# facebookresearch/jepa

Measured on NVIDIA H100. Metric: clips/sec ViT-L/16 16x224^2 synthetic V-JEPA pre-training step, higher is better.
Workload: dtype bf16

## Files before the change

### __graft_entry__.py

```python
import os
import sys

ROOT = os.path.dirname(os.path.abspath(__file__))
if ROOT not in sys.path:
    sys.path.insert(0, ROOT)


def build():
    from jepa_b200 import build as b
    b.build()
    import subprocess
    subprocess.check_call(["make", "-s", "-C", os.path.join(ROOT, "tests", "native"), "all", "test_xattn",
                           "test_gemm_sched"])
    import jepa_b200
    from jepa_b200 import _lib
    _lib.load()
    import oracle.vjepa_oracle


def smoke():
    import torch
    sys.path.insert(0, os.path.join(ROOT, "tests"))
    sys.path.insert(0, os.path.join(ROOT, "tests", "golden"))
    from parity_util import run_c1_step_cuda, run_c1_step_oracle, compare_step
    assert torch.cuda.is_available(), "smoke() needs cuda:0"
    dev = torch.device("cuda:0")
    got = run_c1_step_cuda(dev, batch=1, depth_limit=2)
    ref = run_c1_step_oracle(batch=1, depth_limit=2)
    compare_step(got, ref, verbose=True)
    print("smoke OK: loss", got["loss_jepa"], "oracle", ref["loss_jepa"])


if __name__ == "__main__":
    build()
    if len(sys.argv) > 1 and sys.argv[1] == "smoke":
        smoke()
```

### jepa_b200/csrc/attn_bwd.cu

```cuda
#include <stdlib.h>

#include "attn_common.cuh"
#include "vjepa_b200.h"

namespace vj {

constexpr int kBwdThreads = 384;
constexpr int kBwdStream = 64;
constexpr int kBwdStages = 3;

struct AttnBwdParams {
  const int* cu_seqlens;
  const float* lse2;
  const float* delta;
  __nv_bfloat16* dqkv;
  int H, T;
  float scale, scale_log2;
};

template <int HD>
struct BwdCfg {
  using A = AttnCfg<HD>;
  static constexpr int RES = A::template tile_bytes<128>();
  static constexpr int STR = A::template tile_bytes<kBwdStream>();
  static constexpr int T0 = 0, T1 = RES;
  static constexpr int S_OFF = 2 * RES;
  static constexpr int STAT_OFF = S_OFF + kBwdStages * 2 * STR;
  static constexpr int STAT = 2 * kBwdStream * 4;
  static constexpr int BAR_OFF = STAT_OFF + kBwdStages * STAT;
  static constexpr int SMEM_BYTES = BAR_OFF + 8 * (1 + 2 * kBwdStages) + 1024;
  static_assert(SMEM_BYTES <= 232448, "attention backward shared memory budget exceeded");
};

__global__ void __launch_bounds__(256) attn_delta_kernel(const __nv_bfloat16* __restrict__ o,
                                                         const __nv_bfloat16* __restrict__ dout,
                                                         float* __restrict__ delta, int T, int H, int HD) {
  const int lane = threadIdx.x & 31;
  const int wpb = blockDim.x >> 5;
  const int D = H * HD;
  const int nvec = D >> 3;
  const int lanes_per_head = HD >> 3;
  for (long long t = (long long)blockIdx.x * wpb + (threadIdx.x >> 5); t < T; t += (long long)gridDim.x * wpb) {
    for (int c = lane; c < ((nvec + 31) / 32) * 32; c += 32) {
      float s = 0.f;
      if (c < nvec) {
        const uint4 a = *reinterpret_cast<const uint4*>(o + t * D + c * 8);
        const uint4 b = *reinterpret_cast<const uint4*>(dout + t * D + c * 8);
        s = bf16_lo(a.x) * bf16_lo(b.x) + bf16_hi(a.x) * bf16_hi(b.x) + bf16_lo(a.y) * bf16_lo(b.y) +
            bf16_hi(a.y) * bf16_hi(b.y) + bf16_lo(a.z) * bf16_lo(b.z) + bf16_hi(a.z) * bf16_hi(b.z) +
            bf16_lo(a.w) * bf16_lo(b.w) + bf16_hi(a.w) * bf16_hi(b.w);
      }
      for (int o2 = lanes_per_head >> 1; o2 > 0; o2 >>= 1) s += __shfl_xor_sync(0xffffffffu, s, o2);
      if (c < nvec && (lane % lanes_per_head) == 0) delta[(long long)((c * 8) / HD) * T + t] = s;
    }
  }
}

template <int HD, bool DKV>
__global__ void __launch_bounds__(kBwdThreads, 1)
attn_bwd_kernel(const __grid_constant__ CUtensorMap tmRes, const __grid_constant__ CUtensorMap tmStr,
                const __grid_constant__ CUtensorMap tmDO, const AttnBwdParams p) {
  using B = BwdCfg<HD>;
  extern __shared__ uint8_t smem_raw[];
  uint8_t* smem = reinterpret_cast<uint8_t*>((reinterpret_cast<uintptr_t>(smem_raw) + 1023) & ~uintptr_t(1023));

  const int seq = blockIdx.y, head = blockIdx.z;
  const int row_begin = p.cu_seqlens[seq];
  const int len = p.cu_seqlens[seq + 1] - row_begin;
  const int t0 = blockIdx.x * 128;
  if (t0 >= len) return;
  const int n_it = (len + kBwdStream - 1) / kBwdStream;
  const int HHD = p.H * HD;

  uint64_t* bars = reinterpret_cast<uint64_t*>(smem + B::BAR_OFF);
  const uint32_t bar_res = smem_u32(bars + 0);
  const uint32_t full0 = smem_u32(bars + 1);
  const uint32_t empty0 = smem_u32(bars + 1 + kBwdStages);
  const uint32_t sT0 = smem_u32(smem + B::T0), sT1 = smem_u32(smem + B::T1), sS = smem_u32(smem + B::S_OFF);
  const uint32_t sStat = smem_u32(smem + B::STAT_OFF);
  const float* lse_h = p.lse2 + (long long)head * p.T + row_begin;
  const float* del_h = p.delta + (long long)head * p.T + row_begin;
  const int wg = threadIdx.x >> 7;
  const int lane = threadIdx.x & 31;

  if (threadIdx.x == 0) {
    mbar_init(bar_res, 1);
    for (int st = 0; st < kBwdStages; ++st) {
      mbar_init(full0 + 8 * st, DKV ? 32 : 1);
      mbar_init(empty0 + 8 * st, 8);
    }
    fence_mbar_init();
  }
  __syncthreads();

  if (wg == 0) {
    setmaxnreg_dec<40>();
    if (threadIdx.x < 32) {
      if (lane == 0) {
        mbar_expect_tx(bar_res, 2 * B::RES);
        if (DKV) {
          attn_load_tile<HD, 128>(sT0, &tmRes, bar_res, HHD + head * HD, row_begin + t0);
          attn_load_tile<HD, 128>(sT1, &tmRes, bar_res, 2 * HHD + head * HD, row_begin + t0);
        } else {
          attn_load_tile<HD, 128>(sT0, &tmRes, bar_res, head * HD, row_begin + t0);
          attn_load_tile<HD, 128>(sT1, &tmDO, bar_res, head * HD, row_begin + t0);
        }
      }
      for (int i = 0; i < n_it; ++i) {
        const int st = i % kBwdStages;
        const uint32_t a = sS + st * 2 * B::STR, b = a + B::STR, bar = full0 + 8 * st;
        const int c0 = i * kBwdStream;
        mbar_wait(empty0 + 8 * st, ((i / kBwdStages) & 1) ^ 1);
        if (DKV) {
#pragma unroll
          for (int k = 0; k < kBwdStream / 32; ++k) {
            const int col = c0 + 32 * k + lane;
            const uint32_t dst = sStat + st * B::STAT + (32 * k + lane) * 4;
            sts32f(dst, col < len ? lse_h[col] : 0.f);
            sts32f(dst + B::STAT / 2, col < len ? del_h[col] : 0.f);
          }
        }
        if (lane == 0) {
          mbar_expect_tx(bar, 2 * B::STR);
          if (DKV) {
            attn_load_tile<HD, kBwdStream>(a, &tmStr, bar, head * HD, row_begin + c0);
            attn_load_tile<HD, kBwdStream>(b, &tmDO, bar, head * HD, row_begin + c0);
          } else {
            attn_load_tile<HD, kBwdStream>(a, &tmStr, bar, HHD + head * HD, row_begin + c0);
            attn_load_tile<HD, kBwdStream>(b, &tmStr, bar, 2 * HHD + head * HD, row_begin + c0);
          }
        } else if (DKV) {
          mbar_arrive(bar);
        }
      }
    }
    return;
  }

  setmaxnreg_inc<232>();
  const int cw = wg - 1;
  const int r = cw * 64 + ((threadIdx.x >> 5) & 3) * 16 + (lane >> 2);
  float acc0[HD / 2], acc1[HD / 2];
#pragma unroll
  for (int i = 0; i < HD / 2; ++i) { acc0[i] = 0.f; acc1[i] = 0.f; }
  float row_lse[2], row_del[2];
  if (!DKV) {
#pragma unroll
    for (int h = 0; h < 2; ++h) {
      const int q = t0 + r + 8 * h;
      row_lse[h] = q < len ? lse_h[q] : 0.f;
      row_del[h] = q < len ? del_h[q] : 0.f;
    }
  }
  mbar_wait(bar_res, 0);
  for (int i = 0; i < n_it; ++i) {
    const int st = i % kBwdStages;
    const uint32_t sa = sS + st * 2 * B::STR, sb = sa + B::STR;
    const int c0 = i * kBwdStream;
    mbar_wait(full0 + 8 * st, (i / kBwdStages) & 1);
    float x[kBwdStream / 2], y[kBwdStream / 2];
    wgmma_fence();
#pragma unroll
    for (int kk = 0; kk < HD / 16; ++kk)
      wgmma_ss<kBwdStream, 0, 0>(x, attn_kmajor_desc<HD, 128>(sT0, cw * 64, kk), attn_kmajor_desc<HD, kBwdStream>(sa, 0, kk),
                                 kk > 0);
#pragma unroll
    for (int kk = 0; kk < HD / 16; ++kk)
      wgmma_ss<kBwdStream, 0, 0>(y, attn_kmajor_desc<HD, 128>(sT1, cw * 64, kk), attn_kmajor_desc<HD, kBwdStream>(sb, 0, kk),
                                 kk > 0);
    wgmma_commit();
    wgmma_wait<0>();
    wgmma_fence_regs(x);
    wgmma_fence_regs(y);

#pragma unroll
    for (int c = 0; c < kBwdStream / 8; ++c)
#pragma unroll
      for (int e = 0; e < 2; ++e) {
        const int col = 8 * c + 2 * (lane & 3) + e;
        const bool col_ok = c0 + col < len;
        float cl = 0.f, cd = 0.f;
        if (DKV) {
          cl = lds32f(sStat + st * B::STAT + col * 4);
          cd = lds32f(sStat + st * B::STAT + B::STAT / 2 + col * 4);
        }
#pragma unroll
        for (int h = 0; h < 2; ++h) {
          const float l2 = DKV ? cl : row_lse[h], dl = DKV ? cd : row_del[h];
          float& pv = x[4 * c + 2 * h + e];
          float& dv = y[4 * c + 2 * h + e];
          pv = col_ok ? ex2_approx(fmaf(pv, p.scale_log2, -l2)) : 0.f;
          dv = pv * (dv - dl);
        }
      }

    wgmma_fence_regs(acc0);
    wgmma_fence_regs(acc1);
    wgmma_fence();
#pragma unroll
    for (int kk = 0; kk < kBwdStream / 16; ++kk) {
      uint32_t a[4];
      if (DKV) {
        acc_to_afrag(x, kk, a);
        wgmma_rs<HD, 1>(acc0, a, attn_mnmajor_desc<HD, kBwdStream>(sb, kk), 1);
        acc_to_afrag(y, kk, a);
        wgmma_rs<HD, 1>(acc1, a, attn_mnmajor_desc<HD, kBwdStream>(sa, kk), 1);
      } else {
        acc_to_afrag(y, kk, a);
        wgmma_rs<HD, 1>(acc0, a, attn_mnmajor_desc<HD, kBwdStream>(sa, kk), 1);
      }
    }
    wgmma_commit();
    wgmma_wait<0>();
    wgmma_fence_regs(acc0);
    wgmma_fence_regs(acc1);
    __syncwarp();
    if (lane == 0) mbar_arrive(empty0 + 8 * st);
  }

  __nv_bfloat16* rows = p.dqkv + (long long)(row_begin + t0) * 3 * HHD + head * HD;
  if (DKV) {
    store_frag_bf16<HD>(acc1, p.scale, rows + HHD, 3LL * HHD, r, len - t0);
    store_frag_bf16<HD>(acc0, 1.0f, rows + 2 * HHD, 3LL * HHD, r, len - t0);
  } else {
    store_frag_bf16<HD>(acc0, p.scale, rows, 3LL * HHD, r, len - t0);
  }
}

template <int HD>
static int launch_attn_bwd(const void* qkv, const void* out, const void* dout, const float* lse2, float* delta,
                           void* dqkv, const int* cu, int nseq, int max_len, int H, int T, float scale, cudaStream_t s) {
  using C = AttnCfg<HD>;
  using B = BwdCfg<HD>;
  CUtensorMap tq128, tq64, tdo128, tdo64;
  const uint64_t W = (uint64_t)3 * H * HD;
  int rc = make_tmap_2d(&tq128, qkv, 0, W, T, W * 2, C::BOX_INNER, 128, C::TMAP_SWIZZLE);
  if (!rc) rc = make_tmap_2d(&tq64, qkv, 0, W, T, W * 2, C::BOX_INNER, kBwdStream, C::TMAP_SWIZZLE);
  if (!rc) rc = make_tmap_2d(&tdo128, dout, 0, (uint64_t)H * HD, T, (uint64_t)H * HD * 2, C::BOX_INNER, 128, C::TMAP_SWIZZLE);
  if (!rc) rc = make_tmap_2d(&tdo64, dout, 0, (uint64_t)H * HD, T, (uint64_t)H * HD * 2, C::BOX_INNER, kBwdStream,
                             C::TMAP_SWIZZLE);
  if (rc) return rc;
  auto kdkv = attn_bwd_kernel<HD, true>;
  auto kdq = attn_bwd_kernel<HD, false>;
  static bool configured = false;
  if (!configured) {
    VJ_CUDA(cudaFuncSetAttribute(kdkv, cudaFuncAttributeMaxDynamicSharedMemorySize, B::SMEM_BYTES));
    VJ_CUDA(cudaFuncSetAttribute(kdq, cudaFuncAttributeMaxDynamicSharedMemorySize, B::SMEM_BYTES));
    configured = true;
  }
  {
    int g = (T + 7) / 8;
    const int cap = num_sms() * 8;
    if (g > cap) g = cap;
    attn_delta_kernel<<<g, 256, 0, s>>>(reinterpret_cast<const __nv_bfloat16*>(out),
                                        reinterpret_cast<const __nv_bfloat16*>(dout), delta, T, H, HD);
    VJ_CUDA(cudaGetLastError());
    vj::count_launch(1);
  }
  AttnBwdParams p;
  p.cu_seqlens = cu; p.lse2 = lse2; p.delta = delta; p.dqkv = reinterpret_cast<__nv_bfloat16*>(dqkv);
  p.H = H; p.T = T; p.scale = scale; p.scale_log2 = scale * 1.4426950408889634f;
  dim3 grid((max_len + 127) / 128, nseq, H);
  kdkv<<<grid, kBwdThreads, B::SMEM_BYTES, s>>>(tq128, tq64, tdo64, p);
  VJ_CUDA(cudaGetLastError());
  kdq<<<grid, kBwdThreads, B::SMEM_BYTES, s>>>(tq128, tq64, tdo128, p);
  VJ_CUDA(cudaGetLastError());
  vj::count_launch(2);
  return 0;
}

}

extern "C" int vj_attn_bwd(const void* qkv, const void* out, const void* dout, const float* lse2, float* delta_ws,
                           void* dqkv, float* dq_acc_ws, const int* cu_seqlens, int nseq, int max_len, int H, int HD,
                           int T, float scale, void* stream_) {
  using namespace vj;
  (void)dq_acc_ws;
  cudaStream_t s = reinterpret_cast<cudaStream_t>(stream_);
  VJ_CHECK_ARG(qkv && out && dout && lse2 && delta_ws && dqkv && cu_seqlens, "vj_attn_bwd: null pointer");
  VJ_CHECK_ARG(nseq > 0 && max_len > 0 && H > 0 && T > 0, "vj_attn_bwd: empty problem");
  switch (HD) {
    case 32: return launch_attn_bwd<32>(qkv, out, dout, lse2, delta_ws, dqkv, cu_seqlens, nseq, max_len, H, T, scale, s);
    case 64: return launch_attn_bwd<64>(qkv, out, dout, lse2, delta_ws, dqkv, cu_seqlens, nseq, max_len, H, T, scale, s);
    case 128: return launch_attn_bwd<128>(qkv, out, dout, lse2, delta_ws, dqkv, cu_seqlens, nseq, max_len, H, T, scale, s);
    default: set_error("vj_attn_bwd: head dim %d unsupported (32/64/128)", HD); return -1;
  }
}
```

### jepa_b200/csrc/attn_fwd.cu

```cuda
#include <stdlib.h>

#include "attn_common.cuh"
#include "vjepa_b200.h"

namespace vj {

constexpr int kFwdThreads = 384;
constexpr int kFwdKV = 128;
constexpr int kFwdStages = 3;

struct AttnFwdParams {
  const int* cu_seqlens;
  __nv_bfloat16* out;
  float* lse2;
  int H, T;
  long long ld_out;
  float scale_log2;
};

template <int HD>
struct FwdCfg {
  using A = AttnCfg<HD>;
  static constexpr int TILE = A::template tile_bytes<128>();
  static constexpr int Q_OFF = 0;
  static constexpr int K_OFF = TILE;
  static constexpr int V_OFF = K_OFF + kFwdStages * TILE;
  static constexpr int BAR_OFF = V_OFF + kFwdStages * TILE;
  static constexpr int SMEM_BYTES = BAR_OFF + 8 * (1 + 2 * kFwdStages) + 1024;
  static_assert(SMEM_BYTES <= 232448, "attention forward shared memory budget exceeded");
};

VJ_DEVINL void pingpong_wait_turn(int cw) { named_bar_sync(1 + cw, 256); }
VJ_DEVINL void pingpong_pass_turn(int cw) { named_bar_arrive(2 - cw, 256); }

template <int HD>
__global__ void __launch_bounds__(kFwdThreads, 1)
attn_fwd_kernel(const __grid_constant__ CUtensorMap tmQKV, const AttnFwdParams p) {
  using F = FwdCfg<HD>;
  extern __shared__ uint8_t smem_raw[];
  uint8_t* smem = reinterpret_cast<uint8_t*>((reinterpret_cast<uintptr_t>(smem_raw) + 1023) & ~uintptr_t(1023));

  const int seq = blockIdx.y, head = blockIdx.z;
  const int row_begin = p.cu_seqlens[seq];
  const int len = p.cu_seqlens[seq + 1] - row_begin;
  const int q0 = blockIdx.x * 128;
  if (q0 >= len) return;
  const int n_kv = (len + kFwdKV - 1) / kFwdKV;

  uint64_t* bars = reinterpret_cast<uint64_t*>(smem + F::BAR_OFF);
  const uint32_t bar_q = smem_u32(bars + 0);
  const uint32_t full0 = smem_u32(bars + 1);
  const uint32_t empty0 = smem_u32(bars + 1 + kFwdStages);
  const uint32_t sQ = smem_u32(smem + F::Q_OFF), sK = smem_u32(smem + F::K_OFF), sV = smem_u32(smem + F::V_OFF);
  const int HHD = p.H * HD;
  const int wg = threadIdx.x >> 7;

  if (threadIdx.x == 0) {
    mbar_init(bar_q, 1);
    for (int st = 0; st < kFwdStages; ++st) {
      mbar_init(full0 + 8 * st, 1);
      mbar_init(empty0 + 8 * st, 8);
    }
    fence_mbar_init();
    tma_prefetch_desc(&tmQKV);
  }
  __syncthreads();

  if (wg == 0) {
    setmaxnreg_dec<40>();
    if (threadIdx.x == 0) {
      mbar_expect_tx(bar_q, F::TILE);
      attn_load_tile<HD, 128>(sQ, &tmQKV, bar_q, head * HD, row_begin + q0);
      for (int j = 0; j < n_kv; ++j) {
        const int st = j % kFwdStages;
        mbar_wait(empty0 + 8 * st, ((j / kFwdStages) & 1) ^ 1);
        const uint32_t fb = full0 + 8 * st;
        mbar_expect_tx(fb, 2 * F::TILE);
        attn_load_tile<HD, 128>(sK + st * F::TILE, &tmQKV, fb, HHD + head * HD, row_begin + j * kFwdKV);
        attn_load_tile<HD, 128>(sV + st * F::TILE, &tmQKV, fb, 2 * HHD + head * HD, row_begin + j * kFwdKV);
      }
    }
    return;
  }

  setmaxnreg_inc<232>();
  const int cw = wg - 1;
  const int lane = threadIdx.x & 31;
  const int r = cw * 64 + ((threadIdx.x >> 5) & 3) * 16 + (lane >> 2);
  float o[HD / 2];
#pragma unroll
  for (int i = 0; i < HD / 2; ++i) o[i] = 0.f;
  float m_run[2] = {-INFINITY, -INFINITY}, l_run[2] = {0.f, 0.f};
  float s[kFwdKV / 2];
  uint32_t pf[kFwdKV / 16][4];
  if (cw == 1) pingpong_pass_turn(cw);

  auto issue_s = [&](int st) {
#pragma unroll
    for (int kk = 0; kk < HD / 16; ++kk)
      wgmma_ss<kFwdKV, 0, 0>(s, attn_kmajor_desc<HD, 128>(sQ, cw * 64, kk),
                             attn_kmajor_desc<HD, 128>(sK + st * F::TILE, 0, kk), kk > 0);
    wgmma_commit();
  };
  auto issue_pv = [&](int st) {
#pragma unroll
    for (int kk = 0; kk < kFwdKV / 16; ++kk) wgmma_rs<HD, 1>(o, pf[kk], attn_mnmajor_desc<HD, 128>(sV + st * F::TILE, kk), 1);
    wgmma_commit();
  };
  auto release = [&](int st) {
    __syncwarp();
    if (lane == 0) mbar_arrive(empty0 + 8 * st);
  };
  auto softmax = [&](int j, float (&alpha)[2]) {
    const int valid = len - j * kFwdKV;
    if (valid < kFwdKV) {
#pragma unroll
      for (int c = 0; c < kFwdKV / 8; ++c)
#pragma unroll
        for (int e = 0; e < 4; ++e)
          if (8 * c + 2 * (lane & 3) + (e & 1) >= valid) s[4 * c + e] = -INFINITY;
    }
#pragma unroll
    for (int h = 0; h < 2; ++h) {
      float mx = -INFINITY;
#pragma unroll
      for (int c = 0; c < kFwdKV / 8; ++c)
#pragma unroll
        for (int e = 0; e < 2; ++e) mx = fmaxf(mx, s[4 * c + 2 * h + e]);
      mx = quad_max(mx);
      const float m_new = fmaxf(m_run[h], mx);
      alpha[h] = ex2_approx((m_run[h] - m_new) * p.scale_log2);
      m_run[h] = m_new;
      const float moff = m_new * p.scale_log2;
      float sum = 0.f;
#pragma unroll
      for (int c = 0; c < kFwdKV / 8; ++c)
#pragma unroll
        for (int e = 0; e < 2; ++e) {
          float& v = s[4 * c + 2 * h + e];
          v = ex2_approx(fmaf(v, p.scale_log2, -moff));
          sum += v;
        }
      l_run[h] = l_run[h] * alpha[h] + sum;
    }
  };
  auto rescale_o = [&](const float (&alpha)[2]) {
#pragma unroll
    for (int c = 0; c < HD / 8; ++c) {
      o[4 * c + 0] *= alpha[0]; o[4 * c + 1] *= alpha[0];
      o[4 * c + 2] *= alpha[1]; o[4 * c + 3] *= alpha[1];
    }
  };
  auto pack_p = [&]() {
#pragma unroll
    for (int kk = 0; kk < kFwdKV / 16; ++kk) acc_to_afrag(s, kk, pf[kk]);
  };

  mbar_wait(bar_q, 0);
  float alpha[2];
  pingpong_wait_turn(cw);
  mbar_wait(full0, 0);
  wgmma_fence();
  issue_s(0);
  pingpong_pass_turn(cw);
  wgmma_wait<0>();
  wgmma_fence_regs(s);
  softmax(0, alpha);
  rescale_o(alpha);
  pack_p();
  for (int j = 1; j < n_kv; ++j) {
    const int st = j % kFwdStages, st_prev = (j - 1) % kFwdStages;
    pingpong_wait_turn(cw);
    mbar_wait(full0 + 8 * st, (j / kFwdStages) & 1);
    wgmma_fence_regs(o);
    wgmma_fence();
    issue_s(st);
    issue_pv(st_prev);
    pingpong_pass_turn(cw);
    wgmma_wait<1>();
    wgmma_fence_regs(s);
    softmax(j, alpha);
    wgmma_wait<0>();
    wgmma_fence_regs(o);
    wgmma_fence_regs(pf);
    release(st_prev);
    rescale_o(alpha);
    pack_p();
  }
  pingpong_wait_turn(cw);
  wgmma_fence_regs(o);
  wgmma_fence();
  issue_pv((n_kv - 1) % kFwdStages);
  pingpong_pass_turn(cw);
  wgmma_wait<0>();
  wgmma_fence_regs(o);
  wgmma_fence_regs(pf);
  if (cw == 0) pingpong_wait_turn(cw);

  float inv[2];
#pragma unroll
  for (int h = 0; h < 2; ++h) {
    const float l = quad_sum(l_run[h]);
    inv[h] = 1.0f / l;
    const int row = q0 + r + 8 * h;
    if ((lane & 3) == 0 && row < len) p.lse2[(long long)head * p.T + row_begin + row] = m_run[h] * p.scale_log2 + log2f(l);
  }
#pragma unroll
  for (int c = 0; c < HD / 8; ++c) {
    o[4 * c + 0] *= inv[0]; o[4 * c + 1] *= inv[0];
    o[4 * c + 2] *= inv[1]; o[4 * c + 3] *= inv[1];
  }
  store_frag_bf16<HD>(o, 1.0f, p.out + (long long)(row_begin + q0) * p.ld_out + head * HD, p.ld_out, r, len - q0);
}

template <int HD>
static int launch_attn_fwd(const void* qkv, void* out, float* lse2, const int* cu, int nseq, int max_len, int H, int T,
                           float scale, cudaStream_t s) {
  using C = AttnCfg<HD>;
  using F = FwdCfg<HD>;
  CUtensorMap tm;
  int rc = make_tmap_2d(&tm, qkv, 0, (uint64_t)3 * H * HD, T, (uint64_t)3 * H * HD * 2, C::BOX_INNER, 128,
                        C::TMAP_SWIZZLE);
  if (rc) return rc;
  auto kern = attn_fwd_kernel<HD>;
  static bool configured = false;
  if (!configured) {
    VJ_CUDA(cudaFuncSetAttribute(kern, cudaFuncAttributeMaxDynamicSharedMemorySize, F::SMEM_BYTES));
    configured = true;
  }
  AttnFwdParams p;
  p.cu_seqlens = cu; p.out = reinterpret_cast<__nv_bfloat16*>(out); p.lse2 = lse2;
  p.H = H; p.T = T; p.ld_out = (long long)H * HD;
  p.scale_log2 = scale * 1.4426950408889634f;
  dim3 grid((max_len + 127) / 128, nseq, H);
  kern<<<grid, kFwdThreads, F::SMEM_BYTES, s>>>(tm, p);
  VJ_CUDA(cudaGetLastError());
  vj::count_launch(1);
  return 0;
}

}

extern "C" int vj_attn_fwd(const void* qkv, void* out, float* lse2, const int* cu_seqlens, int nseq, int max_len,
                           int H, int HD, int T, float scale, void* stream_) {
  using namespace vj;
  cudaStream_t s = reinterpret_cast<cudaStream_t>(stream_);
  VJ_CHECK_ARG(qkv && out && lse2 && cu_seqlens, "vj_attn_fwd: null pointer");
  VJ_CHECK_ARG(nseq > 0 && max_len > 0 && H > 0 && T > 0, "vj_attn_fwd: empty problem");
  VJ_CHECK_ARG((reinterpret_cast<uintptr_t>(qkv) & 15) == 0 && (reinterpret_cast<uintptr_t>(out) & 15) == 0,
               "vj_attn_fwd: pointers must be 16-byte aligned");
  switch (HD) {
    case 32: return launch_attn_fwd<32>(qkv, out, lse2, cu_seqlens, nseq, max_len, H, T, scale, s);
    case 64: return launch_attn_fwd<64>(qkv, out, lse2, cu_seqlens, nseq, max_len, H, T, scale, s);
    case 128: return launch_attn_fwd<128>(qkv, out, lse2, cu_seqlens, nseq, max_len, H, T, scale, s);
    default: set_error("vj_attn_fwd: head dim %d unsupported (32/64/128; pad 24->32 in the weights)", HD); return -1;
  }
}
```

Measured before the change: 106.3.

## Make attention forward persistent and drop producer warpgroup in small-head backward

The forward attention kernel becomes persistent: a grid sized to the SM budget loops over (query tile, sequence, head) items, with a new Q-empty barrier so the producer can prefetch the next item's Q and K/V tiles while consumers finish the current one. The backward kernel, for head dim 32, removes the dedicated producer warpgroup and has the first consumer warp issue loads with a lookahead of two stages, allowing two CTAs per SM. This aims to cut tail and launch waste in the forward pass and raise occupancy in the backward pass. In exchange it adds scheduling complexity and a strided item order that may hurt K/V cache locality. Since ViT-L uses head dim 64, the backward change does not run for this workload.

```diff
diff --git a/__graft_entry__.py b/__graft_entry__.py
--- a/__graft_entry__.py
+++ b/__graft_entry__.py
@@ -11,7 +11,7 @@
     b.build()
     import subprocess
     subprocess.check_call(["make", "-s", "-C", os.path.join(ROOT, "tests", "native"), "all", "test_xattn",
-                           "test_gemm_sched"])
+                           "test_gemm_sched", "attn_step"])
     import jepa_b200
     from jepa_b200 import _lib
     _lib.load()
diff --git a/jepa_b200/csrc/attn_bwd.cu b/jepa_b200/csrc/attn_bwd.cu
--- a/jepa_b200/csrc/attn_bwd.cu
+++ b/jepa_b200/csrc/attn_bwd.cu
@@ -5,9 +5,9 @@
 
 namespace vj {
 
-constexpr int kBwdThreads = 384;
 constexpr int kBwdStream = 64;
 constexpr int kBwdStages = 3;
+constexpr int kBwdLookahead = 2;
 
 struct AttnBwdParams {
   const int* cu_seqlens;
@@ -30,6 +30,10 @@
   static constexpr int BAR_OFF = STAT_OFF + kBwdStages * STAT;
   static constexpr int SMEM_BYTES = BAR_OFF + 8 * (1 + 2 * kBwdStages) + 1024;
   static_assert(SMEM_BYTES <= 232448, "attention backward shared memory budget exceeded");
+  static constexpr bool PRODUCER_WG = HD > 32;
+  static constexpr int THREADS = PRODUCER_WG ? 384 : 256;
+  static constexpr int CTAS_PER_SM = PRODUCER_WG ? 1 : 2;
+  static_assert(CTAS_PER_SM * SMEM_BYTES <= 232448, "attention backward: CTAs per SM exceed shared memory");
 };
 
 __global__ void __launch_bounds__(256) attn_delta_kernel(const __nv_bfloat16* __restrict__ o,
@@ -57,7 +61,7 @@
 }
 
 template <int HD, bool DKV>
-__global__ void __launch_bounds__(kBwdThreads, 1)
+__global__ void __launch_bounds__(BwdCfg<HD>::THREADS, BwdCfg<HD>::CTAS_PER_SM)
 attn_bwd_kernel(const __grid_constant__ CUtensorMap tmRes, const __grid_constant__ CUtensorMap tmStr,
                 const __grid_constant__ CUtensorMap tmDO, const AttnBwdParams p) {
   using B = BwdCfg<HD>;
@@ -93,52 +97,78 @@
   }
   __syncthreads();
 
-  if (wg == 0) {
-    setmaxnreg_dec<40>();
-    if (threadIdx.x < 32) {
-      if (lane == 0) {
-        mbar_expect_tx(bar_res, 2 * B::RES);
-        if (DKV) {
-          attn_load_tile<HD, 128>(sT0, &tmRes, bar_res, HHD + head * HD, row_begin + t0);
-          attn_load_tile<HD, 128>(sT1, &tmRes, bar_res, 2 * HHD + head * HD, row_begin + t0);
-        } else {
-          attn_load_tile<HD, 128>(sT0, &tmRes, bar_res, head * HD, row_begin + t0);
-          attn_load_tile<HD, 128>(sT1, &tmDO, bar_res, head * HD, row_begin + t0);
+  auto load_resident = [&]() {
+    if (lane == 0) {
+      mbar_expect_tx(bar_res, 2 * B::RES);
+      if (DKV) {
+        attn_load_tile<HD, 128>(sT0, &tmRes, bar_res, HHD + head * HD, row_begin + t0);
+        attn_load_tile<HD, 128>(sT1, &tmRes, bar_res, 2 * HHD + head * HD, row_begin + t0);
+      } else {
+        attn_load_tile<HD, 128>(sT0, &tmRes, bar_res, head * HD, row_begin + t0);
+        attn_load_tile<HD, 128>(sT1, &tmDO, bar_res, head * HD, row_begin + t0);
+      }
+    }
+  };
+  auto load_stats = [&](int i, float (&sl)[2], float (&sd)[2]) {
+#pragma unroll
+    for (int k = 0; k < kBwdStream / 32; ++k) {
+      const int col = i * kBwdStream + 32 * k + lane;
+      sl[k] = DKV && col < len ? lse_h[col] : 0.f;
+      sd[k] = DKV && col < len ? del_h[col] : 0.f;
+    }
+  };
+  auto load_streamed = [&](int i, const float (&sl)[2], const float (&sd)[2]) {
+    const int st = i % kBwdStages;
+    const uint32_t a = sS + st * 2 * B::STR, b = a + B::STR, bar = full0 + 8 * st;
+    const int c0 = i * kBwdStream;
+    mbar_wait(empty0 + 8 * st, ((i / kBwdStages) & 1) ^ 1);
+    if (DKV) {
+#pragma unroll
+      for (int k = 0; k < kBwdStream / 32; ++k) {
+        const uint32_t dst = sStat + st * B::STAT + (32 * k + lane) * 4;
+        sts32f(dst, sl[k]);
+        sts32f(dst + B::STAT / 2, sd[k]);
+      }
+    }
+    if (lane == 0) {
+      mbar_expect_tx(bar, 2 * B::STR);
+      if (DKV) {
+        attn_load_tile<HD, kBwdStream>(a, &tmStr, bar, head * HD, row_begin + c0);
+        attn_load_tile<HD, kBwdStream>(b, &tmDO, bar, head * HD, row_begin + c0);
+      } else {
+        attn_load_tile<HD, kBwdStream>(a, &tmStr, bar, HHD + head * HD, row_begin + c0);
+        attn_load_tile<HD, kBwdStream>(b, &tmStr, bar, 2 * HHD + head * HD, row_begin + c0);
+      }
+    } else if (DKV) {
+      mbar_arrive(bar);
+    }
+  };
+
+  if constexpr (B::PRODUCER_WG) {
+    if (wg == 0) {
+      setmaxnreg_dec<40>();
+      if (threadIdx.x < 32) {
+        load_resident();
+        for (int i = 0; i < n_it; ++i) {
+          float sl[2], sd[2];
+          load_stats(i, sl, sd);
+          load_streamed(i, sl, sd);
         }
       }
-      for (int i = 0; i < n_it; ++i) {
-        const int st = i % kBwdStages;
-        const uint32_t a = sS + st * 2 * B::STR, b = a + B::STR, bar = full0 + 8 * st;
-        const int c0 = i * kBwdStream;
-        mbar_wait(empty0 + 8 * st, ((i / kBwdStages) & 1) ^ 1);
-        if (DKV) {
-#pragma unroll
-          for (int k = 0; k < kBwdStream / 32; ++k) {
-            const int col = c0 + 32 * k + lane;
-            const uint32_t dst = sStat + st * B::STAT + (32 * k + lane) * 4;
-            sts32f(dst, col < len ? lse_h[col] : 0.f);
-            sts32f(dst + B::STAT / 2, col < len ? del_h[col] : 0.f);
-          }
-        }
-        if (lane == 0) {
-          mbar_expect_tx(bar, 2 * B::STR);
-          if (DKV) {
-            attn_load_tile<HD, kBwdStream>(a, &tmStr, bar, head * HD, row_begin + c0);
-            attn_load_tile<HD, kBwdStream>(b, &tmDO, bar, head * HD, row_begin + c0);
-          } else {
-            attn_load_tile<HD, kBwdStream>(a, &tmStr, bar, HHD + head * HD, row_begin + c0);
-            attn_load_tile<HD, kBwdStream>(b, &tmStr, bar, 2 * HHD + head * HD, row_begin + c0);
-          }
-        } else if (DKV) {
-          mbar_arrive(bar);
-        }
-      }
-    }
-    return;
-  }
-
-  setmaxnreg_inc<232>();
-  const int cw = wg - 1;
+      return;
+    }
+    setmaxnreg_inc<232>();
+  } else if (threadIdx.x < 32) {
+    load_resident();
+    for (int i = 0; i < kBwdLookahead && i < n_it; ++i) {
+      float sl[2], sd[2];
+      load_stats(i, sl, sd);
+      load_streamed(i, sl, sd);
+    }
+  }
+
+  const int cw = B::PRODUCER_WG ? wg - 1 : wg;
+  const bool loader = !B::PRODUCER_WG && threadIdx.x < 32;
   const int r = cw * 64 + ((threadIdx.x >> 5) & 3) * 16 + (lane >> 2);
   float acc0[HD / 2], acc1[HD / 2];
 #pragma unroll
@@ -157,6 +187,9 @@
     const int st = i % kBwdStages;
     const uint32_t sa = sS + st * 2 * B::STR, sb = sa + B::STR;
     const int c0 = i * kBwdStream;
+    const bool load_ahead = loader && i + kBwdLookahead < n_it;
+    float ahead_l[2], ahead_d[2];
+    if (load_ahead) load_stats(i + kBwdLookahead, ahead_l, ahead_d);
     mbar_wait(full0 + 8 * st, (i / kBwdStages) & 1);
     float x[kBwdStream / 2], y[kBwdStream / 2];
     wgmma_fence();
@@ -169,6 +202,7 @@
       wgmma_ss<kBwdStream, 0, 0>(y, attn_kmajor_desc<HD, 128>(sT1, cw * 64, kk), attn_kmajor_desc<HD, kBwdStream>(sb, 0, kk),
                                  kk > 0);
     wgmma_commit();
+    if (load_ahead) load_streamed(i + kBwdLookahead, ahead_l, ahead_d);
     wgmma_wait<0>();
     wgmma_fence_regs(x);
     wgmma_fence_regs(y);
@@ -261,9 +295,9 @@
   p.cu_seqlens = cu; p.lse2 = lse2; p.delta = delta; p.dqkv = reinterpret_cast<__nv_bfloat16*>(dqkv);
   p.H = H; p.T = T; p.scale = scale; p.scale_log2 = scale * 1.4426950408889634f;
   dim3 grid((max_len + 127) / 128, nseq, H);
-  kdkv<<<grid, kBwdThreads, B::SMEM_BYTES, s>>>(tq128, tq64, tdo64, p);
+  kdkv<<<grid, B::THREADS, B::SMEM_BYTES, s>>>(tq128, tq64, tdo64, p);
   VJ_CUDA(cudaGetLastError());
-  kdq<<<grid, kBwdThreads, B::SMEM_BYTES, s>>>(tq128, tq64, tdo128, p);
+  kdq<<<grid, B::THREADS, B::SMEM_BYTES, s>>>(tq128, tq64, tdo128, p);
   VJ_CUDA(cudaGetLastError());
   vj::count_launch(2);
   return 0;
diff --git a/jepa_b200/csrc/attn_fwd.cu b/jepa_b200/csrc/attn_fwd.cu
--- a/jepa_b200/csrc/attn_fwd.cu
+++ b/jepa_b200/csrc/attn_fwd.cu
@@ -13,7 +13,7 @@
   const int* cu_seqlens;
   __nv_bfloat16* out;
   float* lse2;
-  int H, T;
+  int nseq, max_len, H, T;
   long long ld_out;
   float scale_log2;
 };
@@ -26,7 +26,7 @@
   static constexpr int K_OFF = TILE;
   static constexpr int V_OFF = K_OFF + kFwdStages * TILE;
   static constexpr int BAR_OFF = V_OFF + kFwdStages * TILE;
-  static constexpr int SMEM_BYTES = BAR_OFF + 8 * (1 + 2 * kFwdStages) + 1024;
+  static constexpr int SMEM_BYTES = BAR_OFF + 8 * (2 + 2 * kFwdStages) + 1024;
   static_assert(SMEM_BYTES <= 232448, "attention forward shared memory budget exceeded");
 };
 
@@ -40,23 +40,40 @@
   extern __shared__ uint8_t smem_raw[];
   uint8_t* smem = reinterpret_cast<uint8_t*>((reinterpret_cast<uintptr_t>(smem_raw) + 1023) & ~uintptr_t(1023));
 
-  const int seq = blockIdx.y, head = blockIdx.z;
-  const int row_begin = p.cu_seqlens[seq];
-  const int len = p.cu_seqlens[seq + 1] - row_begin;
-  const int q0 = blockIdx.x * 128;
-  if (q0 >= len) return;
-  const int n_kv = (len + kFwdKV - 1) / kFwdKV;
+  const int n_qt = (p.max_len + 127) / 128;
+  const int n_items = n_qt * p.nseq * p.H;
+  const int n_rounds = (n_items + gridDim.x - 1) / gridDim.x;
+  struct Item {
+    bool valid;
+    int head, row_begin, len, q0, n_kv;
+  };
+  auto item = [&](int k) {
+    Item it;
+    const int w = k * gridDim.x + (blockIdx.x + k) % gridDim.x;
+    it.valid = w < n_items;
+    if (!it.valid) return it;
+    const int seq = (w / n_qt) % p.nseq;
+    it.head = w / (n_qt * p.nseq);
+    it.row_begin = p.cu_seqlens[seq];
+    it.len = p.cu_seqlens[seq + 1] - it.row_begin;
+    it.q0 = (w % n_qt) * 128;
+    it.n_kv = (it.len + kFwdKV - 1) / kFwdKV;
+    it.valid = it.q0 < it.len;
+    return it;
+  };
 
   uint64_t* bars = reinterpret_cast<uint64_t*>(smem + F::BAR_OFF);
   const uint32_t bar_q = smem_u32(bars + 0);
-  const uint32_t full0 = smem_u32(bars + 1);
-  const uint32_t empty0 = smem_u32(bars + 1 + kFwdStages);
+  const uint32_t q_empty = smem_u32(bars + 1);
+  const uint32_t full0 = smem_u32(bars + 2);
+  const uint32_t empty0 = smem_u32(bars + 2 + kFwdStages);
   const uint32_t sQ = smem_u32(smem + F::Q_OFF), sK = smem_u32(smem + F::K_OFF), sV = smem_u32(smem + F::V_OFF);
   const int HHD = p.H * HD;
   const int wg = threadIdx.x >> 7;
 
   if (threadIdx.x == 0) {
     mbar_init(bar_q, 1);
+    mbar_init(q_empty, 8);
     for (int st = 0; st < kFwdStages; ++st) {
       mbar_init(full0 + 8 * st, 1);
       mbar_init(empty0 + 8 * st, 8);
@@ -69,15 +86,22 @@
   if (wg == 0) {
     setmaxnreg_dec<40>();
     if (threadIdx.x == 0) {
-      mbar_expect_tx(bar_q, F::TILE);
-      attn_load_tile<HD, 128>(sQ, &tmQKV, bar_q, head * HD, row_begin + q0);
-      for (int j = 0; j < n_kv; ++j) {
-        const int st = j % kFwdStages;
-        mbar_wait(empty0 + 8 * st, ((j / kFwdStages) & 1) ^ 1);
-        const uint32_t fb = full0 + 8 * st;
-        mbar_expect_tx(fb, 2 * F::TILE);
-        attn_load_tile<HD, 128>(sK + st * F::TILE, &tmQKV, fb, HHD + head * HD, row_begin + j * kFwdKV);
-        attn_load_tile<HD, 128>(sV + st * F::TILE, &tmQKV, fb, 2 * HHD + head * HD, row_begin + j * kFwdKV);
+      int n = 0, kv = 0;
+      for (int k = 0; k < n_rounds; ++k) {
+        const Item it = item(k);
+        if (!it.valid) continue;
+        mbar_wait(q_empty, (n & 1) ^ 1);
+        mbar_expect_tx(bar_q, F::TILE);
+        attn_load_tile<HD, 128>(sQ, &tmQKV, bar_q, it.head * HD, it.row_begin + it.q0);
+        for (int j = 0; j < it.n_kv; ++j, ++kv) {
+          const int st = kv % kFwdStages;
+          mbar_wait(empty0 + 8 * st, ((kv / kFwdStages) & 1) ^ 1);
+          const uint32_t fb = full0 + 8 * st;
+          mbar_expect_tx(fb, 2 * F::TILE);
+          attn_load_tile<HD, 128>(sK + st * F::TILE, &tmQKV, fb, HHD + it.head * HD, it.row_begin + j * kFwdKV);
+          attn_load_tile<HD, 128>(sV + st * F::TILE, &tmQKV, fb, 2 * HHD + it.head * HD, it.row_begin + j * kFwdKV);
+        }
+        ++n;
       }
     }
     return;
@@ -88,12 +112,10 @@
   const int lane = threadIdx.x & 31;
   const int r = cw * 64 + ((threadIdx.x >> 5) & 3) * 16 + (lane >> 2);
   float o[HD / 2];
-#pragma unroll
-  for (int i = 0; i < HD / 2; ++i) o[i] = 0.f;
-  float m_run[2] = {-INFINITY, -INFINITY}, l_run[2] = {0.f, 0.f};
+  float m_run[2], l_run[2];
   float s[kFwdKV / 2];
   uint32_t pf[kFwdKV / 16][4];
-  if (cw == 1) pingpong_pass_turn(cw);
+  int len = 0;
 
   auto issue_s = [&](int st) {
 #pragma unroll
@@ -156,61 +178,80 @@
     for (int kk = 0; kk < kFwdKV / 16; ++kk) acc_to_afrag(s, kk, pf[kk]);
   };
 
-  mbar_wait(bar_q, 0);
-  float alpha[2];
-  pingpong_wait_turn(cw);
-  mbar_wait(full0, 0);
-  wgmma_fence();
-  issue_s(0);
-  pingpong_pass_turn(cw);
-  wgmma_wait<0>();
-  wgmma_fence_regs(s);
-  softmax(0, alpha);
-  rescale_o(alpha);
-  pack_p();
-  for (int j = 1; j < n_kv; ++j) {
-    const int st = j % kFwdStages, st_prev = (j - 1) % kFwdStages;
+  if (cw == 1) pingpong_pass_turn(cw);
+  int n = 0, kv = 0;
+  for (int k = 0; k < n_rounds; ++k) {
+    const Item it = item(k);
+    if (!it.valid) continue;
+    len = it.len;
+#pragma unroll
+    for (int i = 0; i < HD / 2; ++i) o[i] = 0.f;
+    m_run[0] = m_run[1] = -INFINITY;
+    l_run[0] = l_run[1] = 0.f;
+
+    mbar_wait(bar_q, n & 1);
+    float alpha[2];
     pingpong_wait_turn(cw);
-    mbar_wait(full0 + 8 * st, (j / kFwdStages) & 1);
+    mbar_wait(full0 + 8 * (kv % kFwdStages), (kv / kFwdStages) & 1);
+    wgmma_fence();
+    issue_s(kv % kFwdStages);
+    pingpong_pass_turn(cw);
+    wgmma_wait<0>();
+    wgmma_fence_regs(s);
+    softmax(0, alpha);
+    rescale_o(alpha);
+    pack_p();
+    for (int j = 1; j < it.n_kv; ++j) {
+      const int st = (kv + j) % kFwdStages, st_prev = (kv + j - 1) % kFwdStages;
+      pingpong_wait_turn(cw);
+      mbar_wait(full0 + 8 * st, ((kv + j) / kFwdStages) & 1);
+      wgmma_fence_regs(o);
+      wgmma_fence();
+      issue_s(st);
+      issue_pv(st_prev);
+      pingpong_pass_turn(cw);
+      wgmma_wait<1>();
+      wgmma_fence_regs(s);
+      softmax(j, alpha);
+      wgmma_wait<0>();
+      wgmma_fence_regs(o);
+      wgmma_fence_regs(pf);
+      release(st_prev);
+      rescale_o(alpha);
+      pack_p();
+    }
+    __syncwarp();
+    if (lane == 0) mbar_arrive(q_empty);
+    kv += it.n_kv;
+    ++n;
+    pingpong_wait_turn(cw);
     wgmma_fence_regs(o);
     wgmma_fence();
-    issue_s(st);
-    issue_pv(st_prev);
+    issue_pv((kv - 1) % kFwdStages);
     pingpong_pass_turn(cw);
-    wgmma_wait<1>();
-    wgmma_fence_regs(s);
-    softmax(j, alpha);
     wgmma_wait<0>();
     wgmma_fence_regs(o);
     wgmma_fence_regs(pf);
-    release(st_prev);
-    rescale_o(alpha);
-    pack_p();
-  }
-  pingpong_wait_turn(cw);
-  wgmma_fence_regs(o);
-  wgmma_fence();
-  issue_pv((n_kv - 1) % kFwdStages);
-  pingpong_pass_turn(cw);
-  wgmma_wait<0>();
-  wgmma_fence_regs(o);
-  wgmma_fence_regs(pf);
+    release((kv - 1) % kFwdStages);
+
+    float inv[2];
+#pragma unroll
+    for (int h = 0; h < 2; ++h) {
+      const float l = quad_sum(l_run[h]);
+      inv[h] = 1.0f / l;
+      const int row = it.q0 + r + 8 * h;
+      if ((lane & 3) == 0 && row < len)
+        p.lse2[(long long)it.head * p.T + it.row_begin + row] = m_run[h] * p.scale_log2 + log2f(l);
+    }
+#pragma unroll
+    for (int c = 0; c < HD / 8; ++c) {
+      o[4 * c + 0] *= inv[0]; o[4 * c + 1] *= inv[0];
+      o[4 * c + 2] *= inv[1]; o[4 * c + 3] *= inv[1];
+    }
+    store_frag_bf16<HD>(o, 1.0f, p.out + (long long)(it.row_begin + it.q0) * p.ld_out + it.head * HD, p.ld_out, r,
+                        len - it.q0);
+  }
   if (cw == 0) pingpong_wait_turn(cw);
-
-  float inv[2];
-#pragma unroll
-  for (int h = 0; h < 2; ++h) {
-    const float l = quad_sum(l_run[h]);
-    inv[h] = 1.0f / l;
-    const int row = q0 + r + 8 * h;
-    if ((lane & 3) == 0 && row < len) p.lse2[(long long)head * p.T + row_begin + row] = m_run[h] * p.scale_log2 + log2f(l);
-  }
-#pragma unroll
-  for (int c = 0; c < HD / 8; ++c) {
-    o[4 * c + 0] *= inv[0]; o[4 * c + 1] *= inv[0];
-    o[4 * c + 2] *= inv[1]; o[4 * c + 3] *= inv[1];
-  }
-  store_frag_bf16<HD>(o, 1.0f, p.out + (long long)(row_begin + q0) * p.ld_out + head * HD, p.ld_out, r, len - q0);
 }
 
 template <int HD>
@@ -230,9 +271,11 @@
   }
   AttnFwdParams p;
   p.cu_seqlens = cu; p.out = reinterpret_cast<__nv_bfloat16*>(out); p.lse2 = lse2;
-  p.H = H; p.T = T; p.ld_out = (long long)H * HD;
+  p.nseq = nseq; p.max_len = max_len; p.H = H; p.T = T; p.ld_out = (long long)H * HD;
   p.scale_log2 = scale * 1.4426950408889634f;
-  dim3 grid((max_len + 127) / 128, nseq, H);
+  const long long items = (long long)((max_len + 127) / 128) * nseq * H;
+  VJ_CHECK_ARG(items < (1LL << 30), "vj_attn_fwd: too many (query tile, sequence, head) items");
+  const int grid = items < sm_budget() ? (int)items : sm_budget();
   kern<<<grid, kFwdThreads, F::SMEM_BYTES, s>>>(tm, p);
   VJ_CUDA(cudaGetLastError());
   vj::count_launch(1);
```

Result: faster. 108.2 (median of 6 runs) (+1.7%).
